# zju3dv/OnePose_Plus_Plus

Hardware: AMD Instinct MI355X
Metric: query images/sec (2D-3D match fwd) at 512x512 img x 5k pts (higher is better)
Workload: dtype f32 (operands as exact bf16 triples, f32 accumulate)

## Files before the change

### onepose_plus_plus_amd/build.py

```python
import hashlib
import os
import subprocess
import sys
from concurrent.futures import ThreadPoolExecutor

HERE = os.path.dirname(os.path.abspath(__file__))
CSRC = os.path.join(HERE, "csrc")
OBJ = os.path.join(HERE, "csrc", "_build")
LIB = os.path.join(HERE, "libopp_hip.so")
SOURCES = ["gemm_mfma.hip", "gemm_ss.hip", "enc_chain.hip", "enc_layer64.hip", "stem_direct.hip", "attention.hip", "full_attention.hip", "backbone.hip", "kpt.hip",
           "coarse_match.hip", "fine.hip", "pnp.hip", "pnp_batch.hip", "pnp_lo.hip", "pnp_lo_batch.hip", "pose_metrics.hip", "ingest.hip", "track.hip", "profile.hip", "bn_train.hip", "bankbuild.hip", "loss.hip", "linear_bwd.hip",
           "linattn_train.hip", "conv_bwd.hip", "train_misc.hip", "conv_tail.hip", "version.hip", "api.hip"]
HEADERS = ["opp_common.h", "opp_internal.h", "enc_frag.h", "pnp_math.h", "pnp_sample.h", "pnp_body.h", "pnp_batch.h", "pnp_lo_body.h", "pnp_lo_batch.h", os.path.join("..", "..", "include", "opp_hip.h")]
FLAGS = ["--offload-arch=gfx950", "-O3", "-std=c++17", "-fPIC", "-Wall", "-Wno-unused-function"]
SOURCE_FLAGS = {"conv_bwd.hip": ["-fno-slp-vectorize"], "gemm_mfma.hip": ["-fno-slp-vectorize"], "full_attention.hip": ["-fno-slp-vectorize"]}


def _hipcc():
    for cand in (os.environ.get("HIPCC"), "/opt/rocm/bin/hipcc", "hipcc"):
        if cand and (os.path.isabs(cand) and os.path.exists(cand) or not os.path.isabs(cand)):
            return cand
    return "hipcc"


def _max_jobs():
    if os.environ.get("MAX_JOBS", "").isdigit() and int(os.environ["MAX_JOBS"]) > 0:
        return int(os.environ["MAX_JOBS"])
    return len(os.sched_getaffinity(0)) if hasattr(os, "sched_getaffinity") else (os.cpu_count() or 4)


def source_hash():
    h = hashlib.sha256()
    for rel in sorted(SOURCES + HEADERS):
        path = os.path.join(CSRC, rel)
        if not os.path.exists(path):
            return None
        h.update(os.path.basename(rel).encode() + b"\0")
        with open(path, "rb") as f:
            h.update(f.read())
        h.update(b"\0")
    return h.hexdigest()


def _stale(target, deps):
    if not os.path.exists(target):
        return True
# ... 70 lines not shown
```

### onepose_plus_plus_amd/csrc/api.hip

```cpp
#include <math.h>
#include <stdarg.h>

#include <string>
#include <vector>

#include "../../include/opp_hip.h"
#include "opp_internal.h"

static thread_local char g_err[512] = "";
void opp_set_error(const char* fmt, ...) {
  va_list ap;
  va_start(ap, fmt);
  vsnprintf(g_err, sizeof(g_err), fmt, ap);
  va_end(ap);
}
extern "C" const char* opp_last_error(void) { return g_err; }
extern "C" int opp_version(void) { return 1; }

namespace {

inline int pad32(int c) { return (c + 31) / 32 * 32; }

inline int gemm_prec(const opp_config& cfg) {
  return cfg.gemm_precision == 3 ? OPP_PREC_BF16X3 : cfg.gemm_precision ? OPP_PREC_FP16X2 : OPP_PREC_FP32;
// ... 588 lines not shown
  }
};
bool conv_splits_by_shape(const ConvDesc& d, size_t pixels, int prec) {
  return prec == OPP_PREC_BF16X3 && opp_conv_splitk_by_shape((long long)pixels, d.cout_pad(), d.k_len());
}

inline bool asp_env_on() {
  const char* e = getenv("OPP_ASP");
  return e && e[0] == '1';
}
thread_local bool t_asp_on = false;
struct AspScope {
  bool prev;
  AspScope() : prev(t_asp_on) { t_asp_on = asp_env_on(); }
  explicit AspScope(bool on) : prev(t_asp_on) { t_asp_on = on; }
  ~AspScope() { t_asp_on = prev; }
};
bool conv_takes_split(const ConvDesc& d, int prec) {
  return t_asp_on && prec == OPP_PREC_BF16X3 && opp_conv_tail_grp(d.cin, d.ks) == 0 && !(t_conv_tail && d.w_tail != nullptr);
}
inline size_t split_row_bytes(int c_pad) { return (size_t)c_pad * 6; }

inline int conv_out(int in, int ks, int stride, int pad = -1) { return (in + 2 * (pad < 0 ? ks / 2 : pad) - ks) / stride + 1; }

struct ConvOpts {
  int tile_cfg = -1;
  int Bn = 1;
  bool raw = false;
  int pad = -1;
  int splitk_force = -1;
  const void* x3 = nullptr;
  void* y3 = nullptr;
};

int run_conv(const float* x, int Hin, int Win, const ConvDesc& d, int stride, const float* res, int res_mode, int act,
             float* y, hipStream_t s, int h2, const ConvOpts& o = ConvOpts()) {
  OppGemm g;
  const bool raw = o.raw;
  const bool a_split = o.x3 != nullptr && !raw && conv_takes_split(d, h2);
  OPP_CHECK_ARG(a_split || x != nullptr, "conv: no fp32 input for a convolution that cannot take the pre-split one");
  OPP_CHECK_ARG(o.y3 == nullptr || h2 == OPP_PREC_BF16X3, "conv: pre-split output is a bf16x3 feature");
  static const bool splitk_on = !(getenv("OPP_CONV_SPLITK") && getenv("OPP_CONV_SPLITK")[0] == '0');
  g.splitk_ws = splitk_on ? t_splitk_ws : nullptr;
  g.splitk_ws_floats = g.splitk_ws ? t_splitk_ws_floats : 0;
  g.splitk_force = o.splitk_force;
  g.nonfinite = t_status_flag;
  g.tile_policy = t_tile_policy;
  g.conv = 1;
  g.prec = h2;
  const float* h2s = raw ? d.h2s_train : d.h2s;
  g.h2_inv = (h2 == OPP_PREC_FP16X2 && h2s) ? h2s + 1 : nullptr;
  g.A0 = a_split ? static_cast<const float*>(o.x3) : x;
  g.a_split = a_split ? 1 : 0;
  g.C3 = o.y3;
  g.ld3 = (int)split_row_bytes(d.cout_pad());
  g.Bn = o.Bn;
  g.Hin = Hin;
  g.Win = Win;
  g.Cin = d.cin_pad();
  g.ksize = d.ks;
  g.stride = stride;
  g.pad = o.pad < 0 ? d.ks / 2 : o.pad;
  g.Hout = conv_out(Hin, d.ks, stride, g.pad);
  g.Wout = conv_out(Win, d.ks, stride, g.pad);
  g.W = raw ? d.w_train : d.w;
  g.K = d.k_len();
  g.tail_grp = opp_conv_tail_grp(d.cin, d.ks);
  g.ldw = (int)split_floats((size_t)g.K, h2);
  g.M = o.Bn * g.Hout * g.Wout;
  g.N = d.cout_pad();
  g.C = y;
  g.ldc = d.cout_pad();
  g.n_store = d.cout_pad();
  g.n_real = d.cout;
  g.bias = raw ? nullptr : d.bias;
  g.res_mode = res_mode;
  g.R = res;
  g.ldr = d.cout_pad();
  if (res_mode == OPP_RES_BILINEAR2X) {
    g.Hr = g.Hout / 2;
    g.Wr = g.Wout / 2;
    g.res_sy = g.Hout > 1 ? (float)(g.Hr - 1) / (float)(g.Hout - 1) : 0.f;
    g.res_sx = g.Wout > 1 ? (float)(g.Wr - 1) / (float)(g.Wout - 1) : 0.f;
  }
  g.act = act;
  g.alg_flops = 2.0 * (double)g.M * (double)d.cout * (double)(d.ks * d.ks * d.cin);
  const float* wt = raw ? d.w_tail_train : d.w_tail;
  if (t_conv_tail && h2 == OPP_PREC_BF16X3 && wt != nullptr && o.tile_cfg < 0) {
    OppGemm body = g;
    body.N = d.body_cols();
    body.n_store = d.body_cols();
    body.alg_flops = 2.0 * (double)g.M * (double)d.body_cols() * (double)(d.ks * d.ks * d.cin);
    OPP_TRY(opp_gemm_launch_cfg(body, o.tile_cfg, s));
    return opp_conv_tail(g, wt, d.body_cols(), d.tail_cols(), s);
  }
  return opp_gemm_launch_cfg(g, o.tile_cfg, s);
}

struct BlockTwins {
  const void* x3 = nullptr;
  void *tmp3 = nullptr, *y3 = nullptr;
};

int run_block(const float* x, int Hin, int Win, const BlockDesc& b, int stride, float* tmp, float* ds, float* y,
              hipStream_t s, int h2, const BlockTwins& tw = BlockTwins()) {
  const int Ho = Hin / stride, Wo = Win / stride;
  const bool t_split = tw.tmp3 != nullptr && conv_takes_split(b.conv2, h2);
  OPP_TRY(run_conv(x, Hin, Win, b.conv1, stride, nullptr, OPP_RES_NONE, OPP_ACT_RELU, t_split ? nullptr : tmp, s, h2,
                   {.x3 = tw.x3, .y3 = t_split ? tw.tmp3 : nullptr}));
  const float* shortcut = x;
  if (b.has_down) {
    OPP_TRY(run_conv(x, Hin, Win, b.down, stride, nullptr, OPP_RES_NONE, OPP_ACT_NONE, ds, s, h2, {.x3 = tw.x3}));
    shortcut = ds;
  }
  OPP_CHECK_ARG(shortcut != nullptr, "block: the shortcut needs the fp32 input map");
  return run_conv(t_split ? nullptr : tmp, Ho, Wo, b.conv2, 1, shortcut, OPP_RES_DIRECT, OPP_ACT_RELU, y, s, h2,
                  {.x3 = t_split ? tw.tmp3 : nullptr, .y3 = tw.y3});
}

struct BackboneBufs {
  float *col, *x0, *t1, *x1a, *x1, *t2, *ds2, *x2a, *x2, *t3, *ds3, *x3a, *x3, *l2, *u2, *x2o, *l1, *u1;
  float *sk1 = nullptr, *sk2 = nullptr;
  void *x0s = nullptr, *t1s = nullptr, *x1as = nullptr, *x1s = nullptr, *x2s = nullptr, *t3s = nullptr, *x3as = nullptr, *x3s = nullptr, *l2s = nullptr,
       *u2s = nullptr;
};

size_t plan_backbone(const opp_ctx* c, int B, int H, int W, bool infer, Arena& a, BackboneBufs& b) {
  const size_t p2 = (size_t)B * (H / 2) * (W / 2), p4 = (size_t)B * (H / 4) * (W / 4), p8 = (size_t)B * (H / 8) * (W / 8);
// ... 1683 lines not shown
```

### onepose_plus_plus_amd/csrc/gemm_mfma.hip

```cpp
#include <stdlib.h>

#include <mutex>
#include <type_traits>

#include <vector>

#include "opp_internal.h"

typedef float f32x16 __attribute__((ext_vector_type(16)));
typedef _Float16 f16x8 __attribute__((ext_vector_type(8)));
typedef __bf16 bf16x8 __attribute__((ext_vector_type(8)));
typedef __bf16 bf16x2 __attribute__((ext_vector_type(2)));
typedef float f32x2 __attribute__((ext_vector_type(2)));

namespace {

constexpr int lds_stride(int prec) { return prec == OPP_PREC_BF16X3 ? 52 : 36; }

__device__ __forceinline__ void opp_split4_b3(const float4 v, uint2& hi, uint2& mid, uint2& lo) {
  auto lvl = [](float a, float b, float& ra, float& rb) -> unsigned {
    const f32x2 t = {a, b};
    const unsigned p = __builtin_bit_cast(unsigned, __builtin_convertvector(t, bf16x2));
    ra = a - __uint_as_float(p << 16);
    rb = b - __uint_as_float(p & 0xffff0000u);
    return p;
  };
  float r0, r1, r2, r3, s0, s1, s2, s3, u0, u1, u2, u3;
  const unsigned h01 = lvl(v.x, v.y, r0, r1), h23 = lvl(v.z, v.w, r2, r3);
  const unsigned m01 = lvl(r0, r1, s0, s1), m23 = lvl(r2, r3, s2, s3);
  const unsigned l01 = lvl(s0, s1, u0, u1), l23 = lvl(s2, s3, u2, u3);
  hi = make_uint2(h01, h23);
  mid = make_uint2(m01, m23);
  lo = make_uint2(l01, l23);
}
__device__ __forceinline__ void opp_store_split4(void* base, size_t row_bytes_off, int col, const float4 v) {
  uint2 hi, mid, lo;
  opp_split4_b3(v, hi, mid, lo);
  char* p = static_cast<char*>(base) + row_bytes_off + (col >> 3) * 48 + (col & 7) * 2;
  *reinterpret_cast<uint2*>(p) = hi;
  *reinterpret_cast<uint2*>(p + 16) = mid;
  *reinterpret_cast<uint2*>(p + 32) = lo;
}

template <int BM, int BN, int WAVES_M, int WAVES_N, bool CONV, int ABL, int DEPTH, int PREC, bool ASP, bool KFOLD = false>
__device__ __forceinline__ void opp_gemm_body(const OppGemm& g) {
  constexpr bool H2 = PREC == OPP_PREC_FP16X2;
  constexpr bool H3 = PREC == OPP_PREC_BF16X3;
  constexpr int kLdsStride = lds_stride(PREC);
  constexpr int NT = WAVES_M * WAVES_N * 64;
  constexpr int TM = BM / WAVES_M / 32;
  constexpr int NT32 = BN / 32;
  constexpr int TN = (NT32 + WAVES_N - 1) / WAVES_N;
  constexpr bool kRagged = (NT32 % WAVES_N) != 0;
  static_assert(!ASP || (CONV && PREC == OPP_PREC_BF16X3 && (ABL == 0 || ABL >= 200)), "pre-split activations: bf16x3 convolutions only");
  constexpr int kAblMask = ABL >= 200 ? ABL - 200 : 0;
  constexpr bool kNoGload = ABL == 91 || (kAblMask & 1), kNoLdsSt = ABL == 92 || (kAblMask & 2), kNoBar = ABL == 93 || (kAblMask & 4),
                 kNoFrag = ABL == 94 || (kAblMask & 8);
  constexpr int A_LD = ASP ? (BM * 12 + NT - 1) / NT : BM * 8 / NT;
  constexpr bool kAFrac = ASP && (BM * 12) % NT != 0;
  constexpr int kBRowsLoad = (H3 && BN == 224) ? 208 : BN;
  constexpr int B_LD = H3 ? (kBRowsLoad * 12 + NT - 1) / NT : BN * 8 / NT;
  constexpr bool kBFrac = H3 && (kBRowsLoad * 12) % NT != 0;
  constexpr bool kRing = H3 && kRagged && !CONV;
  constexpr bool kM16 = H3 && CONV;
  constexpr int NB16 = kM16 ? kBRowsLoad / 16 : 1;
  constexpr int NBW = kM16 ? (NB16 + WAVES_N - 1) / WAVES_N : 1;
  constexpr bool kRoles = kM16 && BM == 128 && BN == 224 && WAVES_M == 2 && WAVES_N == 4;
// ... 1076 lines not shown
      if constexpr (decltype(vec_c)::value) return *reinterpret_cast<const vf4*>(p);
      return vf4{p[0], nval > 1 ? p[1] : 0.f, nval > 2 ? p[2] : 0.f, nval > 3 ? p[3] : 0.f};
    };
    auto epi_col = [&](int lc, int& col) __attribute__((always_inline)) -> bool {
      const int wn2 = lc / (JP * 32);
      const int j = ps * JP + (lc - wn2 * JP * 32) / 32;
      col = kM16 ? n0 + lc : n0 + wn2 * TN * 32 + j * 32 + (lc & 31);
      return !((!kM16 && (j >= TN || (kRagged && wn2 * TN + j >= NT32))) || col >= g.n_store);
    };
    vf4 bias_t = vf4{0.f, 0.f, 0.f, 0.f};
    if constexpr (kColFixed) {
      int col;
      if (g.bias && epi_col((tid % kRowQ) * 4, col)) bias_t = vec_ok ? ld4(std::true_type{}, g.bias + col, 4) : ld4(std::false_type{}, g.bias + col, g.n_store - col);
    }
    const bool row_masked = g.act == OPP_ACT_QKV && g.row_mask != nullptr;
    auto epi_load = [&](auto vec_c, auto m_c, int u, EpiItem& it) __attribute__((always_inline)) {
      constexpr int M = decltype(m_c)::value;
      constexpr bool direct = M == kRDirect, bilinear = CONV && M == kRBil;
      it.ok = false;
      if (u >= kUnits) return;
      const int lr = u / kRowQ;
      const int lc = (u - lr * kRowQ) * 4;
      it.row = m0 + lr;
      if (!epi_col(lc, it.col) || it.row >= g.M) return;
      it.ok = true;
      const int nval = g.n_store - it.col < 4 ? g.n_store - it.col : 4;
      it.cv = *reinterpret_cast<const vf4*>(Cs + lr * CS + lc);
      if constexpr (!kColFixed) {
        if (g.bias) it.bv = ld4(vec_c, g.bias + it.col, nval);
      }
      if (row_masked && it.row < g.row_mask_rows) it.rm = g.row_mask[it.row];
      if (direct) it.rd = ld4(vec_c, g.R + (size_t)it.row * g.ldr + it.col, nval);
      if (bilinear) {
#pragma clang fp contract(off)
        const int ox = it.row % g.Wout;
        const int t = it.row / g.Wout;
        const int oy = t % g.Hout;
        const int b = t / g.Hout;
        const float sy = g.res_sy * (float)oy;
        const float sx = g.res_sx * (float)ox;
        int y0 = (int)sy;
        if (y0 > g.Hr - 1) y0 = g.Hr - 1;
        int x0 = (int)sx;
        if (x0 > g.Wr - 1) x0 = g.Wr - 1;
        const int y1 = y0 + (y0 < g.Hr - 1 ? 1 : 0);
        const int x1 = x0 + (x0 < g.Wr - 1 ? 1 : 0);
        it.wy1 = fminf(fmaxf(sy - (float)y0, 0.f), 1.f);
        it.wx1 = fminf(fmaxf(sx - (float)x0, 0.f), 1.f);
        it.wy0 = 1.f - it.wy1;
        it.wx0 = 1.f - it.wx1;
        const int pb = b * g.Hr * g.Wr;
        it.r[0] = ld4(vec_c, g.R + (size_t)(pb + y0 * g.Wr + x0) * g.ldr + it.col, nval);
        it.r[1] = ld4(vec_c, g.R + (size_t)(pb + y0 * g.Wr + x1) * g.ldr + it.col, nval);
        it.r[2] = ld4(vec_c, g.R + (size_t)(pb + y1 * g.Wr + x0) * g.ldr + it.col, nval);
        it.r[3] = ld4(vec_c, g.R + (size_t)(pb + y1 * g.Wr + x1) * g.ldr + it.col, nval);
      }
    };
    auto epi_finish = [&](auto vec_c, auto m_c, auto w_c, const EpiItem& it) __attribute__((always_inline)) {
      constexpr int M = decltype(m_c)::value;
      constexpr bool direct = M == kRDirect, bilinear = CONV && M == kRBil;
      if (!it.ok) return;
      const int row = it.row, col = it.col;
      const int nval = g.n_store - col < 4 ? g.n_store - col : 4;
      float v[4] = {it.cv.x, it.cv.y, it.cv.z, it.cv.w};
      if (g.bias) {
        const vf4 bv = kColFixed ? bias_t : it.bv;
        v[0] += bv.x; v[1] += bv.y; v[2] += bv.z; v[3] += bv.w;
      }
      if (direct) {
        const vf4 rv = it.rd;
        v[0] += rv.x; v[1] += rv.y; v[2] += rv.z; v[3] += rv.w;
      } else if (bilinear) {
#pragma clang fp contract(off)
        const float a00[4] = {it.r[0].x, it.r[0].y, it.r[0].z, it.r[0].w}, a01[4] = {it.r[1].x, it.r[1].y, it.r[1].z, it.r[1].w};
        const float a10[4] = {it.r[2].x, it.r[2].y, it.r[2].z, it.r[2].w}, a11[4] = {it.r[3].x, it.r[3].y, it.r[3].z, it.r[3].w};
#pragma unroll
        for (int e = 0; e < 4; ++e) {
          const float top = it.wx0 * a00[e] + it.wx1 * a01[e];
          const float bot = it.wx0 * a10[e] + it.wx1 * a11[e];
          v[e] += it.wy0 * top + it.wy1 * bot;
        }
      }
      if (g.act == OPP_ACT_RELU) {
#pragma unroll
        for (int e = 0; e < 4; ++e) v[e] = v[e] < 0.f ? 0.f : v[e];
      } else if (g.act == OPP_ACT_LEAKY) {
#pragma unroll
        for (int e = 0; e < 4; ++e) v[e] = v[e] > 0.f ? v[e] : 0.01f * v[e];
      } else if (g.act == OPP_ACT_QKV) {
        if (col < g.qk_cols) {
#pragma unroll
          for (int e = 0; e < 4; ++e) v[e] = v[e] > 0.f ? v[e] + 1.f : __expf(v[e]);
        } else {
          const float vdiv = row < g.split_row ? g.s0 : g.s1;
#pragma unroll
          for (int e = 0; e < 4; ++e) v[e] = v[e] / vdiv;
        }
        if constexpr (decltype(w_c)::value) {
          if (row_masked && row < g.row_mask_rows) {
#pragma unroll
            for (int e = 0; e < 4; ++e) v[e] *= it.rm;
          }
        }
      }
      if constexpr (H3) {
        if (g.C3 != nullptr) opp_store_split4(g.C3, (size_t)row * g.ld3, col, make_float4(v[0], v[1], v[2], v[3]));
      }
      if (g.C == nullptr) return;
      float* cp = g.C + (size_t)row * g.ldc + col + (g.k_splits > 1 ? (size_t)blockIdx.y * g.split_stride : 0);
      if constexpr (decltype(vec_c)::value) {
        *reinterpret_cast<float4*>(cp) = make_float4(v[0], v[1], v[2], v[3]);
      } else {
        for (int e = 0; e < nval; ++e) cp[e] = v[e];
      }
    };
    constexpr int kWaitVm0 = 0x0F70;
    auto epi_batches = [&](auto vec_c, auto eb_c, auto m_c, auto w_c) __attribute__((always_inline)) {
      constexpr int EB = decltype(eb_c)::value;
      constexpr bool W = decltype(w_c)::value;
      if constexpr (!W) __builtin_amdgcn_s_waitcnt(kWaitVm0);
      for (int ub = tid; ub < kUnits; ub += NT * EB) {
        EpiItem it[EB];
// ... 490 lines not shown
```

### onepose_plus_plus_amd/csrc/opp_internal.h

```cpp
#pragma once
#include "opp_common.h"

enum {
  OPP_PROF_FIRST_NON_GEMM = 1000,
  OPP_PROF_LINATTN_KV = 1000,
  OPP_PROF_LINATTN_APPLY = 1001,
  OPP_PROF_CONF = 1002,
  OPP_PROF_FINE = 1003,
  OPP_PROF_LINATTN_SMALL = 1004,
  OPP_PROF_FINE_GATHER = 1005,
  OPP_PROF_FINE_HEAD = 1006,
  OPP_PROF_FOCAL_FWD = 1007,
  OPP_PROF_FOCAL_BWD = 1008,
  OPP_PROF_ENC_CHAIN = 1009,
  OPP_PROF_SCORE_SWEEP1 = 1010,
  OPP_PROF_SCORE_SWEEP2 = 1011,
  OPP_PROF_CONV_WGRAD = 1013,
  OPP_PROF_CONV_SPLITK = 1014,
  OPP_PROF_CONV_TAIL = 1017,
  OPP_PROF_LINATTN_REDUCE = 1016,
  OPP_PROF_SPLITK_EPILOGUE = 1015,
  OPP_PROF_SCORE_SS = 1012,
};
inline int opp_prof_gemm_symbol(int tile_cfg, int kind) { return kind * 256 + tile_cfg; }
struct OppProfScope {
  OppProfScope(int symbol, hipStream_t stream, double work);
  ~OppProfScope();
  OppProfScope(const OppProfScope&) = delete;
  OppProfScope& operator=(const OppProfScope&) = delete;

 private:
  hipStream_t stream_;
  long long slot_ = -1;
};

int opp_layernorm(const float* x, int ldx, const float* gamma, const float* beta, const float* res, int ldres,
                  float* out, int ldo, int rows, int C, float eps, hipStream_t stream);
int opp_linattn_chunks(int seg_len);
int opp_linattn_kv(const float* k, const float* v, int ld, int n_seg, int seg_len, int C, int D, float* kv_out,
                   float* ks_out, float* scratch, hipStream_t stream);
int opp_linattn_apply(const float* q, int ldq, const float* kv, const float* ks, float* out, int ldo, int n_seg,
                      int seg_len, int src_len, int C, int D, float eps, hipStream_t stream);
size_t opp_linattn_pair_scratch_floats(int len0, int len1);
int opp_linattn_kv_pair(const float* qkv, int ld, int len0, int len1, float* kv, float* ks, float* scratch,
                        hipStream_t stream);
void opp_linattn_chunk_parts(float* scratch, int len0, int len1, float** kv_part, float** ks_part);
int opp_linattn_reduce_chunks(int len0, int len1, float* kv, float* ks, float* scratch, hipStream_t stream);
size_t opp_focal_loss_ws_bytes(size_t n);
int opp_focal_loss_fwd(const float* conf, const short* gt, const float* weight, size_t n, float alpha, float gamma, double* sums,
                       void* ws, size_t ws_bytes, hipStream_t stream);
int opp_focal_loss_bwd(const float* conf, const short* gt, const float* weight, size_t n, float alpha, float gamma,
                       const float* scales, float* grad, hipStream_t stream);
int opp_focal_loss_fwd_ex(const float* conf, const void* gt, int gt_kind, const float* weight, const float* mask0, const float* mask1, int N, int L,
                          size_t n, float alpha, float gamma, double* sums, void* ws, size_t ws_bytes, hipStream_t stream);
// ... 61 lines not shown
  const float* rstat_max = nullptr;
  const float* rstat_sum = nullptr;
  const float* cstat_max = nullptr;
  const float* cstat_sum = nullptr;
  float* C = nullptr;
  int ldc = 0;
  float* part_best = nullptr;
  int* part_arg = nullptr;
  int* part_ties = nullptr;
  float* part_rowmax = nullptr;
  int a_bytes = 0, b_bytes = 0, vec_store = 0;
  int delay = 0;
  unsigned long long* dbg_ts = nullptr;
};
void opp_gemm_ss_debug_timestamps(void* buf, int mode);
int opp_gemm_ss_tile_rows();
int opp_gemm_ss_tile_cols();
int opp_gemm_ss(const OppGemmSS& g, hipStream_t stream);
size_t opp_linear_bwd_ws_bytes(int M, int N, int K, int prec);
int opp_linear_bwd(const float* dY, const float* X, const float* W, int M, int N, int K, float* dX, float* dW, int accumulate_dw, int prec,
                   void* ws, size_t ws_bytes, hipStream_t stream);
size_t opp_linattn_train_ws_bytes(int B, int L, int S, int H, int D);
int opp_linattn_train_fwd(const float* q, const float* k, const float* v, const float* q_mask, const float* kv_mask, int B, int L, int S, int H, int D,
                          float eps, float* out, float* kv, float* ks, void* ws, size_t ws_bytes, hipStream_t stream);
int opp_linattn_train_bwd(const float* q, const float* k, const float* v, const float* q_mask, const float* kv_mask, const float* kv, const float* ks,
                          const float* grad_out, int B, int L, int S, int H, int D, float eps, float* gq, float* gk, float* gv, void* ws,
                          size_t ws_bytes, hipStream_t stream);
bool opp_stem_direct_ok(int cout, int prec);
int opp_stem_direct(const float* img, int H, int W, const float* wsplit, const float* bias, float* out, int ldc, hipStream_t stream, void* out3 = nullptr,
                    int ld3 = 0);
size_t opp_conv_tail_weight_floats(int cin_pad, int ks);
int opp_pack_conv_tail(const float* w, const float* scale, int cout, int cin, int ks, int n0, int cin_pad, float* wt, hipStream_t stream);
int opp_conv_tail(const OppGemm& g, const float* wt, int n0, int ncols, hipStream_t stream);
int opp_fold_bn(const float* gamma, const float* beta, const float* mean, const float* var, float eps, int c,
                int c_pad, float* scale, float* shift, hipStream_t stream);
int opp_pack_conv(const float* w, const float* scale, int cout, int cin, int ks, int cout_pad, int cin_pad,
                  float* out, hipStream_t stream);
int opp_pack_stem(const float* w, const float* scale, int cout, float* out, hipStream_t stream);
int opp_stem_im2col(const float* img, int B, int H, int W, float* col, hipStream_t stream);
int opp_h2_split(const float* in, float* out, size_t n, float* scale2, hipStream_t stream);
int opp_b3_split(const float* in, float* out, size_t n, hipStream_t stream);
int opp_add(const float* a, const float* b, float* out, size_t n, hipStream_t stream);
int opp_pack_affine(const float* src, float fill, const float* scale1, float* out, int n, hipStream_t stream);
int opp_add_cat(const float* a, const float* b, size_t na, const float* c, size_t nc, float* out, hipStream_t stream);
int opp_transpose(const float* in, float* out, int batch, int R, int Cc, hipStream_t stream);
size_t opp_bn_train_scratch_bytes(int rows, int ld);
int opp_bn_train(const float* y, int rows, int ld, int C, const float* gamma, const float* beta, float eps, const float* res,
                 int act, float* out, float* stat_out, void* scratch, hipStream_t stream, float* save_mean = nullptr, float* save_invstd = nullptr);
size_t opp_conv_geo_entries(int P);
int opp_conv_geo(int B, int Ho, int Wo, int Hin, int Win, int ks, int stride, int pad, void* geo, hipStream_t stream);
size_t opp_conv_wgrad_ws_bytes(int P, int cout_pad, int cin_pad, int ks);
int opp_conv_wgrad(const float* dY, int ldy, const float* X, int ldx, size_t x_pixels, const void* geo, int P, int Win, int ks, int cout, int cin,
                   float* dW, int accumulate, void* ws, size_t ws_bytes, hipStream_t stream);
int opp_conv_flip_transpose(const float* w, int cout, int cin, int ks, float* out, hipStream_t stream);
int opp_conv_dilate2(const float* dy, int B, int Ho, int Wo, int ld, float* z, hipStream_t stream);
size_t opp_bn_bwd_scratch_bytes(int rows, int ld);
int opp_bn_backward(const float* dy, const float* y, const float* raw, int rows, int ld, int C, int act, const float* gamma, const float* mean,
                    const float* invstd, float* draw, float* dres, float* dgamma, float* dbeta, int accumulate, void* scratch, hipStream_t stream);
int opp_upsample2x_backward(const float* g, int B, int Hr, int Wr, int ld, float* dr, int accumulate, hipStream_t stream);
int opp_ln_forward(const float* x, const float* gamma, const float* beta, const float* res, int rows, int C, float eps, float* y, float* mean,
                   float* rstd, hipStream_t stream);
size_t opp_ln_backward_ws_bytes(int rows, int C);
int opp_ln_backward(const float* g, const float* x, const float* gamma, const float* mean, const float* rstd, int rows, int C, float* dx,
                    float* dgamma, float* dbeta, void* ws, size_t ws_bytes, hipStream_t stream);
size_t opp_lse_ws_bytes(int B, int N, int L);
int opp_dual_softmax_lse(const float* S, int B, int N, int L, float* lse_row, float* lse_col, float* conf, void* ws, size_t ws_bytes,
// ... 38 lines not shown
```

Measured before the change: 597.0.

## Add dedicated short-K 1x1 convolution MFMA kernel for bf16x3 convs

Result: no change. 596.5 (-0.1%).

```diff
diff --git a/onepose_plus_plus_amd/build.py b/onepose_plus_plus_amd/build.py
--- a/onepose_plus_plus_amd/build.py
+++ b/onepose_plus_plus_amd/build.py
@@ -10,8 +10,8 @@
 LIB = os.path.join(HERE, "libopp_hip.so")
 SOURCES = ["gemm_mfma.hip", "gemm_ss.hip", "enc_chain.hip", "enc_layer64.hip", "stem_direct.hip", "attention.hip", "full_attention.hip", "backbone.hip", "kpt.hip",
            "coarse_match.hip", "fine.hip", "pnp.hip", "pnp_batch.hip", "pnp_lo.hip", "pnp_lo_batch.hip", "pose_metrics.hip", "ingest.hip", "track.hip", "profile.hip", "bn_train.hip", "bankbuild.hip", "loss.hip", "linear_bwd.hip",
-           "linattn_train.hip", "conv_bwd.hip", "train_misc.hip", "conv_tail.hip", "version.hip", "api.hip"]
-HEADERS = ["opp_common.h", "opp_internal.h", "enc_frag.h", "pnp_math.h", "pnp_sample.h", "pnp_body.h", "pnp_batch.h", "pnp_lo_body.h", "pnp_lo_batch.h", os.path.join("..", "..", "include", "opp_hip.h")]
+           "linattn_train.hip", "conv_bwd.hip", "train_misc.hip", "conv_tail.hip", "conv1x1.hip", "version.hip", "api.hip"]
+HEADERS = ["opp_common.h", "opp_internal.h", "conv_epilogue.h", "split_b3.h", "enc_frag.h", "pnp_math.h", "pnp_sample.h", "pnp_body.h", "pnp_batch.h", "pnp_lo_body.h", "pnp_lo_batch.h", os.path.join("..", "..", "include", "opp_hip.h")]
 FLAGS = ["--offload-arch=gfx950", "-O3", "-std=c++17", "-fPIC", "-Wall", "-Wno-unused-function"]
 SOURCE_FLAGS = {"conv_bwd.hip": ["-fno-slp-vectorize"], "gemm_mfma.hip": ["-fno-slp-vectorize"], "full_attention.hip": ["-fno-slp-vectorize"]}
 
diff --git a/onepose_plus_plus_amd/csrc/api.hip b/onepose_plus_plus_amd/csrc/api.hip
--- a/onepose_plus_plus_amd/csrc/api.hip
+++ b/onepose_plus_plus_amd/csrc/api.hip
@@ -644,6 +644,11 @@
   const void* x3 = nullptr;
   void* y3 = nullptr;
 };
+
+inline int conv1x1_mode() {
+  const char* v = getenv("OPP_CONV1X1");
+  return v && (v[0] == '0' || v[0] == '1') ? v[0] - '0' : -1;
+}
 
 int run_conv(const float* x, int Hin, int Win, const ConvDesc& d, int stride, const float* res, int res_mode, int act,
              float* y, hipStream_t s, int h2, const ConvOpts& o = ConvOpts()) {
@@ -706,6 +711,10 @@
     OPP_TRY(opp_gemm_launch_cfg(body, o.tile_cfg, s));
     return opp_conv_tail(g, wt, d.body_cols(), d.tail_cols(), s);
   }
+  const int c1_mode = conv1x1_mode();
+  if (o.tile_cfg < 0 && !raw && o.x3 == nullptr && o.y3 == nullptr && h2 == OPP_PREC_BF16X3 && c1_mode != 0 &&
+      (c1_mode == 1 || g.M < opp_conv1x1_max_pixels()) && opp_conv1x1_takes(g))
+    return opp_conv1x1_launch(g, s);
   return opp_gemm_launch_cfg(g, o.tile_cfg, s);
 }
 
diff --git a/onepose_plus_plus_amd/csrc/conv1x1.hip b/onepose_plus_plus_amd/csrc/conv1x1.hip
--- /dev/null
+++ b/onepose_plus_plus_amd/csrc/conv1x1.hip
@@ -0,0 +1,276 @@
+#include <stdlib.h>
+
+#include <type_traits>
+
+#include "conv_epilogue.h"
+#include "opp_internal.h"
+#include "split_b3.h"
+
+namespace {
+
+typedef __bf16 bf16x8 __attribute__((ext_vector_type(8)));
+typedef float f32x4 __attribute__((ext_vector_type(4)));
+typedef unsigned int u32x4 __attribute__((ext_vector_type(4)));
+
+constexpr int kTileM = 64;
+constexpr int kNT = 256;
+constexpr int kRowF = 52;
+constexpr int kFill = 4;
+constexpr int kChunkF = kTileM * kRowF;
+constexpr unsigned kOob = 0x80000000u;
+
+__device__ __forceinline__ int c1_kswz(int r) { return ((r >> 2) ^ (r >> 3)) & 1; }
+__device__ __forceinline__ float4 c1_bload(const __amdgpu_buffer_rsrc_t r, unsigned voff, unsigned soff) {
+  const u32x4 v = __builtin_amdgcn_raw_buffer_load_b128(r, (int)voff, (int)soff, 0);
+  return make_float4(__uint_as_float(v.x), __uint_as_float(v.y), __uint_as_float(v.z), __uint_as_float(v.w));
+}
+__device__ __forceinline__ bf16x8 c1_b8(const float4& v) { return *reinterpret_cast<const bf16x8*>(&v); }
+
+__global__ __launch_bounds__(kNT, 3) void conv1x1_kernel(const OppGemm g, const int nb_comp) {
+  __shared__ __attribute__((aligned(16))) float As[kFill * kChunkF];
+
+  const int tid = threadIdx.x;
+  const int lane = tid & 63;
+  const int wave = __builtin_amdgcn_readfirstlane(tid >> 6);
+  int tile = blockIdx.x;
+  {
+    const int nb = gridDim.x, q = nb >> 3, r = nb & 7;
+    const int xcd = blockIdx.x & 7, idx = blockIdx.x >> 3;
+    tile = (xcd < r ? xcd * (q + 1) : r * (q + 1) + (xcd - r) * q) + idx;
+  }
+  const int m0 = tile * kTileM;
+  const int nk = g.K >> 5;
+
+  const int role = (wave + tile) & 3;
+  const int wg_base = nb_comp / (int)gridDim.y, wg_rem = nb_comp % (int)gridDim.y;
+  const int wg_nb = wg_base + ((int)blockIdx.y < wg_rem ? 1 : 0);
+  const int wg_cb0 = (int)blockIdx.y * wg_base + ((int)blockIdx.y < wg_rem ? (int)blockIdx.y : wg_rem);
+  const int nb_base = wg_nb >> 2, nb_rem = wg_nb & 3;
+  const int nbw = nb_base + (role < nb_rem ? 1 : 0);
+  const int cb0 = wg_cb0 + role * nb_base + (role < nb_rem ? role : nb_rem);
+
+  const int kq = tid & 7, lrow = tid >> 3;
+  unsigned a_base[2];
+  int a_lds[2];
+#pragma unroll
+  for (int h = 0; h < 2; ++h) {
+    const int lr = lrow + 32 * h;
+    const int r = m0 + lr;
+    const int ox = r % g.Wout;
+    const int t = r / g.Wout;
+    const int oy = t % g.Hout;
+    const int b = t / g.Hout;
+    a_base[h] = r < g.M ? (unsigned)(((b * g.Hin + oy * g.stride) * g.Win + ox * g.stride) * g.Cin + kq * 4) * 4u : kOob;
+    a_lds[h] = lr * kRowF + ((kq >> 1) ^ c1_kswz(lr)) * 12 + (kq & 1) * 2;
+  }
+  const __amdgpu_buffer_rsrc_t ra = __builtin_amdgcn_make_buffer_rsrc(const_cast<float*>(g.A0), 0, g.a0_bytes, 0x00020000);
+  const __amdgpu_buffer_rsrc_t rw = __builtin_amdgcn_make_buffer_rsrc(const_cast<float*>(g.W), 0, g.w_bytes, 0x00020000);
+  auto stage = [&](int c0, auto grp_c) __attribute__((always_inline)) {
+    constexpr int G = decltype(grp_c)::value;
+#pragma unroll
+    for (int c1 = 0; c1 < kFill; c1 += G) {
+      float4 v[G][2];
+#pragma unroll
+      for (int ci = 0; ci < G; ++ci)
+#pragma unroll
+        for (int h = 0; h < 2; ++h) v[ci][h] = c1_bload(ra, (c0 + c1 + ci < nk ? a_base[h] : kOob) + (unsigned)(c0 + c1 + ci) * 128u, 0);
+#pragma unroll
+      for (int ci = 0; ci < G; ++ci)
+#pragma unroll
+        for (int h = 0; h < 2; ++h) {
+          uint2 hi, mid, lo;
+          opp_split4_b3(v[ci][h], hi, mid, lo);
+          float* dst = As + (c1 + ci) * kChunkF + a_lds[h];
+          *reinterpret_cast<uint2*>(dst) = hi;
+          *reinterpret_cast<uint2*>(dst + 4) = mid;
+          *reinterpret_cast<uint2*>(dst + 8) = lo;
+        }
+    }
+  };
+
+  const int l15 = lane & 15, kg = lane >> 4;
+  const int f16off = l15 * kRowF + ((kg ^ c1_kswz(l15)) * 3) * 4;
+  const unsigned w_voff = (unsigned)((cb0 * 16 + l15) * g.ldw) * 4u + (unsigned)kg * 48u;
+  const unsigned w_blk = (unsigned)(16 * g.ldw) * 4u;
+
+  auto body = [&](auto nbw_c) __attribute__((always_inline)) {
+    constexpr int NBW = decltype(nbw_c)::value;
+    constexpr int NBA = NBW > 0 ? NBW : 1;
+    constexpr int WD = NBW <= 1 ? 8 : NBW == 2 ? 3 : NBW == 3 ? 2 : 1;
+    f32x4 acc[4][NBA];
+    float4 wf[WD][NBA][3];
+    float4 af[2][3];
+#pragma unroll
+    for (int i = 0; i < 4; ++i)
+#pragma unroll
+      for (int j = 0; j < NBA; ++j) acc[i][j] = f32x4{0.f, 0.f, 0.f, 0.f};
+    auto load_w = [&](int slot, int j, int c) {
+      const int cc = c < nk ? c : nk - 1;
+#pragma unroll
+      for (int p = 0; p < 3; ++p) wf[slot][j][p] = c1_bload(rw, w_voff, (unsigned)j * w_blk + (unsigned)cc * 192u + (unsigned)p * 16u);
+    };
+    auto read_a = [&](int slot, const float* img, int i) {
+#pragma unroll
+      for (int p = 0; p < 3; ++p) af[slot][p] = *reinterpret_cast<const float4*>(img + i * 16 * kRowF + p * 4);
+    };
+    auto chunk = [&](auto c_c) __attribute__((always_inline)) {
+      constexpr int CC = decltype(c_c)::value, SLOT = CC % WD;
+      constexpr int PA[6] = {2, 0, 1, 1, 0, 0};
+      constexpr int PB[6] = {0, 2, 1, 0, 1, 0};
+      const float* img = As + (CC & (kFill - 1)) * kChunkF + f16off;
+      if (NBW > 0) read_a(0, img, 0);
+#pragma unroll
+      for (int j = 0; j < NBW; ++j) {
+#pragma unroll
+        for (int i = 0; i < 4; ++i) {
+          if (i < 3 || j + 1 < NBW) read_a((i + 1) & 1, img, (i + 1) & 3);
+#pragma unroll
+          for (int pr = 0; pr < 6; ++pr)
+            acc[i][j] = __builtin_amdgcn_mfma_f32_16x16x32_bf16(c1_b8(wf[SLOT][j][PB[pr]]), c1_b8(af[i & 1][PA[pr]]), acc[i][j], 0, 0, 0);
+        }
+        if constexpr (CC + WD < 8) load_w(SLOT, j, CC + WD);
+        __builtin_amdgcn_sched_barrier(0);
+      }
+    };
+
+#pragma unroll
+    for (int sl = 0; sl < WD; ++sl)
+#pragma unroll
+      for (int j = 0; j < NBW; ++j) load_w(sl, j, sl);
+    stage(0, std::integral_constant<int, 4>{});
+    __syncthreads();
+    chunk(std::integral_constant<int, 0>{});
+    chunk(std::integral_constant<int, 1>{});
+    chunk(std::integral_constant<int, 2>{});
+    chunk(std::integral_constant<int, 3>{});
+    if (nk > kFill) {
+      __syncthreads();
+      stage(kFill, std::integral_constant<int, 2>{});
+      __syncthreads();
+      chunk(std::integral_constant<int, 4>{});
+      if (nk > 5) chunk(std::integral_constant<int, 5>{});
+      if (nk > 6) chunk(std::integral_constant<int, 6>{});
+      if (nk > 7) chunk(std::integral_constant<int, 7>{});
+    }
+
+    const opp_vf4 zero4 = opp_vf4{0.f, 0.f, 0.f, 0.f};
+    const opp_vf4 none4[4] = {zero4, zero4, zero4, zero4};
+#pragma unroll
+    for (int j = 0; j < NBW; ++j) {
+      const opp_vf4 bv = g.bias ? *reinterpret_cast<const opp_vf4*>(g.bias + (cb0 + j) * 16 + kg * 4) : zero4;
+#pragma unroll
+      for (int i = 0; i < 4; ++i) {
+        float v[4] = {acc[i][j][0], acc[i][j][1], acc[i][j][2], acc[i][j][3]};
+        opp_epi_bias_res4<false, false>(v, g.bias != nullptr, bv, zero4, none4, 0.f, 0.f, 0.f, 0.f);
+        acc[i][j] = f32x4{v[0], v[1], v[2], v[3]};
+      }
+    }
+    auto finish = [&](auto bil_c) __attribute__((always_inline)) {
+      constexpr bool BIL = decltype(bil_c)::value;
+      auto item = [&](const f32x4 a, const opp_vf4 (&r)[4], const OppBil2x& t, int row, int col) {
+        float v[4] = {a[0], a[1], a[2], a[3]};
+        opp_epi_bias_res4<false, BIL>(v, false, zero4, zero4, r, t.wx0, t.wx1, t.wy0, t.wy1);
+        opp_epi_act4(v, g.act);
+        if (row < g.M) *reinterpret_cast<float4*>(g.C + (size_t)row * g.ldc + col) = make_float4(v[0], v[1], v[2], v[3]);
+      };
+      auto taps = [&](opp_vf4 (&r)[4], const OppBil2x& t, int col) {
+        if constexpr (BIL) {
+          r[0] = *reinterpret_cast<const opp_vf4*>(g.R + (size_t)t.p00 * g.ldr + col);
+          r[1] = *reinterpret_cast<const opp_vf4*>(g.R + (size_t)t.p01 * g.ldr + col);
+          r[2] = *reinterpret_cast<const opp_vf4*>(g.R + (size_t)t.p10 * g.ldr + col);
+          r[3] = *reinterpret_cast<const opp_vf4*>(g.R + (size_t)t.p11 * g.ldr + col);
+        }
+      };
+      auto geo = [&](int i, OppBil2x& t) {
+        const int row = m0 + i * 16 + l15;
+        if constexpr (BIL) opp_epi_bil2x(g, row < g.M ? row : g.M - 1, t);
+      };
+      constexpr int JP = NBW > 0 ? (NBW + 1) / 2 : 1, NBATCH = NBW > 0 ? 4 * JP : 0;
+      OppBil2x t[2] = {};
+      opp_vf4 r[2][2][4];
+      auto request = [&](int b) {
+        const int i = b / JP, j0 = (b % JP) * 2;
+        if (b % JP == 0) geo(i, t[i & 1]);
+#pragma unroll
+        for (int jj = 0; jj < 2; ++jj)
+          if (j0 + jj < NBW) taps(r[b & 1][jj], t[i & 1], (cb0 + j0 + jj) * 16 + kg * 4);
+      };
+      if (NBATCH > 0) request(0);
+#pragma unroll
+      for (int b = 0; b < NBATCH; ++b) {
+        if (b + 1 < NBATCH) request(b + 1);
+        const int i = b / JP, j0 = (b % JP) * 2;
+#pragma unroll
+        for (int jj = 0; jj < 2; ++jj)
+          if (j0 + jj < NBW) item(acc[i][j0 + jj], r[b & 1][jj], t[i & 1], m0 + i * 16 + l15, (cb0 + j0 + jj) * 16 + kg * 4);
+      }
+      if (blockIdx.y == 0) {
+        const int nb_store = g.n_store >> 4;
+        for (int e = nb_comp + wave; e < nb_store; e += 4) {
+          const int col = e * 16 + kg * 4;
+          const opp_vf4 bz = g.bias ? *reinterpret_cast<const opp_vf4*>(g.bias + col) : zero4;
+          for (int i = 0; i < 4; ++i) {
+            OppBil2x tz = {};
+            geo(i, tz);
+            opp_vf4 rz[4];
+            taps(rz, tz, col);
+            float v[4] = {0.f, 0.f, 0.f, 0.f};
+            opp_epi_bias_res4<false, false>(v, g.bias != nullptr, bz, zero4, none4, 0.f, 0.f, 0.f, 0.f);
+            item(f32x4{v[0], v[1], v[2], v[3]}, rz, tz, m0 + i * 16 + l15, col);
+          }
+        }
+      }
+    };
+    if (g.res_mode == OPP_RES_BILINEAR2X) finish(std::true_type{});
+    else finish(std::false_type{});
+  };
+
+  if (nbw == 4) body(std::integral_constant<int, 4>{});
+  else if (nbw == 3) body(std::integral_constant<int, 3>{});
+  else if (nbw == 2) body(std::integral_constant<int, 2>{});
+  else if (nbw == 1) body(std::integral_constant<int, 1>{});
+  else body(std::integral_constant<int, 0>{});
+}
+
+bool al16(const void* p) { return (reinterpret_cast<uintptr_t>(p) & 15) == 0; }
+
+}
+
+int opp_conv1x1_max_pixels() { return 4096; }
+
+bool opp_conv1x1_takes(const OppGemm& g) {
+  if (!g.conv || g.ksize != 1 || g.pad != 0 || (g.stride != 1 && g.stride != 2) || g.prec != OPP_PREC_BF16X3) return false;
+  if (g.a_split || g.C3 != nullptr || g.C == nullptr || g.Bn != 1 || g.k_splits > 1 || g.splitk_force > 0 || g.tail_grp != 0) return false;
+  if (g.K != g.Cin || g.K % 32 != 0 || g.K < 4 * 32 || g.K > 8 * 32) return false;
+  if (g.N <= 0 || g.N % 16 != 0 || g.N > g.n_store || g.n_store > 256 || g.n_store % 16 != 0 || g.ldc < g.n_store || g.ldc % 4 != 0) return false;
+  if (g.res_mode != OPP_RES_NONE && g.res_mode != OPP_RES_BILINEAR2X) return false;
+  if (g.act != OPP_ACT_NONE && g.act != OPP_ACT_RELU && g.act != OPP_ACT_LEAKY) return false;
+  if (g.out_mul != 1.f || g.out_div != 1.f || g.ln_gamma || g.stat_rowmax || g.col_mask || g.row_mask) return false;
+  if (g.M <= 0 || g.M != g.Hout * g.Wout || (size_t)g.M * (size_t)g.ldc >= (1ull << 31)) return false;
+  if ((size_t)g.Hin * g.Win * g.Cin * 4 >= (1ull << 31) || (size_t)g.N * g.ldw * 4 >= (1ull << 31) || g.ldw * 2 < g.K * 3 || g.ldw % 4 != 0) return false;
+  if ((g.Hout - 1) * g.stride >= g.Hin || (g.Wout - 1) * g.stride >= g.Win) return false;
+  if (!al16(g.A0) || !al16(g.W) || !al16(g.C) || !al16(g.bias)) return false;
+  if (g.res_mode == OPP_RES_BILINEAR2X) {
+    if (g.R == nullptr || !al16(g.R) || g.ldr % 4 != 0 || g.ldr < g.n_store || g.Hr <= 0 || g.Wr <= 0) return false;
+    const uintptr_t r0 = reinterpret_cast<uintptr_t>(g.R), r1 = r0 + ((size_t)(g.Hr * g.Wr - 1) * g.ldr + g.n_store) * 4;
+    const uintptr_t c0 = reinterpret_cast<uintptr_t>(g.C), c1 = c0 + ((size_t)(g.M - 1) * g.ldc + g.n_store) * 4;
+    if (!(r1 <= c0 || c1 <= r0)) return false;
+  }
+  return true;
+}
+
+int opp_conv1x1_launch(const OppGemm& g_in, hipStream_t stream) {
+  OPP_CHECK_ARG(opp_conv1x1_takes(g_in), "conv1x1: not a convolution of the short-K kernel");
+  OppGemm g = g_in;
+  g.a0_bytes = (unsigned)((size_t)g.Hin * g.Win * g.Cin * 4);
+  g.w_bytes = (unsigned)((size_t)g.N * g.ldw * 4);
+  const int n_real = g.n_real > 0 && g.n_real < g.N ? g.n_real : g.N;
+  const int nb_comp = (n_real + 15) / 16;
+  OppProfScope prof(OPP_PROF_CONV1X1, stream, g.alg_flops > 0.0 ? g.alg_flops : 2.0 * (double)g.M * (double)g.N * (double)g.K);
+  const int tiles_m = opp_cdiv(g.M, kTileM);
+  int col_split = 1;
+  while (col_split < 4 && tiles_m * col_split < 512 && nb_comp >= 8 * col_split) col_split *= 2;
+  hipLaunchKernelGGL(conv1x1_kernel, dim3(tiles_m, col_split), dim3(kNT), 0, stream, g, nb_comp);
+  OPP_CHECK_LAUNCH("conv1x1_kernel");
+  return OPP_OK;
+}
diff --git a/onepose_plus_plus_amd/csrc/conv_epilogue.h b/onepose_plus_plus_amd/csrc/conv_epilogue.h
--- /dev/null
+++ b/onepose_plus_plus_amd/csrc/conv_epilogue.h
@@ -0,0 +1,66 @@
+#pragma once
+#include "opp_common.h"
+
+#ifdef __HIPCC__
+typedef float opp_vf4 __attribute__((ext_vector_type(4)));
+
+struct OppBil2x {
+  int p00, p01, p10, p11;
+  float wx0, wx1, wy0, wy1;
+};
+__device__ __forceinline__ void opp_epi_bil2x(const OppGemm& g, int row, OppBil2x& t) {
+#pragma clang fp contract(off)
+  const int ox = row % g.Wout;
+  const int q = row / g.Wout;
+  const int oy = q % g.Hout;
+  const int b = q / g.Hout;
+  const float sy = g.res_sy * (float)oy;
+  const float sx = g.res_sx * (float)ox;
+  int y0 = (int)sy;
+  if (y0 > g.Hr - 1) y0 = g.Hr - 1;
+  int x0 = (int)sx;
+  if (x0 > g.Wr - 1) x0 = g.Wr - 1;
+  const int y1 = y0 + (y0 < g.Hr - 1 ? 1 : 0);
+  const int x1 = x0 + (x0 < g.Wr - 1 ? 1 : 0);
+  t.wy1 = fminf(fmaxf(sy - (float)y0, 0.f), 1.f);
+  t.wx1 = fminf(fmaxf(sx - (float)x0, 0.f), 1.f);
+  t.wy0 = 1.f - t.wy1;
+  t.wx0 = 1.f - t.wx1;
+  const int pb = b * g.Hr * g.Wr;
+  t.p00 = pb + y0 * g.Wr + x0;
+  t.p01 = pb + y0 * g.Wr + x1;
+  t.p10 = pb + y1 * g.Wr + x0;
+  t.p11 = pb + y1 * g.Wr + x1;
+}
+
+template <bool DIRECT, bool BILINEAR>
+__device__ __forceinline__ void opp_epi_bias_res4(float (&v)[4], bool has_bias, const opp_vf4 bv, const opp_vf4 rd, const opp_vf4 (&r)[4], float wx0,
+                                                  float wx1, float wy0, float wy1) {
+  if (has_bias) {
+    v[0] += bv.x; v[1] += bv.y; v[2] += bv.z; v[3] += bv.w;
+  }
+  if (DIRECT) {
+    v[0] += rd.x; v[1] += rd.y; v[2] += rd.z; v[3] += rd.w;
+  } else if (BILINEAR) {
+#pragma clang fp contract(off)
+    const float a00[4] = {r[0].x, r[0].y, r[0].z, r[0].w}, a01[4] = {r[1].x, r[1].y, r[1].z, r[1].w};
+    const float a10[4] = {r[2].x, r[2].y, r[2].z, r[2].w}, a11[4] = {r[3].x, r[3].y, r[3].z, r[3].w};
+#pragma unroll
+    for (int e = 0; e < 4; ++e) {
+      const float top = wx0 * a00[e] + wx1 * a01[e];
+      const float bot = wx0 * a10[e] + wx1 * a11[e];
+      v[e] += wy0 * top + wy1 * bot;
+    }
+  }
+}
+
+__device__ __forceinline__ void opp_epi_act4(float (&v)[4], int act) {
+  if (act == OPP_ACT_RELU) {
+#pragma unroll
+    for (int e = 0; e < 4; ++e) v[e] = v[e] < 0.f ? 0.f : v[e];
+  } else if (act == OPP_ACT_LEAKY) {
+#pragma unroll
+    for (int e = 0; e < 4; ++e) v[e] = v[e] > 0.f ? v[e] : 0.01f * v[e];
+  }
+}
+#endif
diff --git a/onepose_plus_plus_amd/csrc/gemm_mfma.hip b/onepose_plus_plus_amd/csrc/gemm_mfma.hip
--- a/onepose_plus_plus_amd/csrc/gemm_mfma.hip
+++ b/onepose_plus_plus_amd/csrc/gemm_mfma.hip
@@ -5,7 +5,9 @@
 
 #include <vector>
 
+#include "conv_epilogue.h"
 #include "opp_internal.h"
+#include "split_b3.h"
 
 typedef float f32x16 __attribute__((ext_vector_type(16)));
 typedef _Float16 f16x8 __attribute__((ext_vector_type(8)));
@@ -17,22 +19,6 @@
 
 constexpr int lds_stride(int prec) { return prec == OPP_PREC_BF16X3 ? 52 : 36; }
 
-__device__ __forceinline__ void opp_split4_b3(const float4 v, uint2& hi, uint2& mid, uint2& lo) {
-  auto lvl = [](float a, float b, float& ra, float& rb) -> unsigned {
-    const f32x2 t = {a, b};
-    const unsigned p = __builtin_bit_cast(unsigned, __builtin_convertvector(t, bf16x2));
-    ra = a - __uint_as_float(p << 16);
-    rb = b - __uint_as_float(p & 0xffff0000u);
-    return p;
-  };
-  float r0, r1, r2, r3, s0, s1, s2, s3, u0, u1, u2, u3;
-  const unsigned h01 = lvl(v.x, v.y, r0, r1), h23 = lvl(v.z, v.w, r2, r3);
-  const unsigned m01 = lvl(r0, r1, s0, s1), m23 = lvl(r2, r3, s2, s3);
-  const unsigned l01 = lvl(s0, s1, u0, u1), l23 = lvl(s2, s3, u2, u3);
-  hi = make_uint2(h01, h23);
-  mid = make_uint2(m01, m23);
-  lo = make_uint2(l01, l23);
-}
 __device__ __forceinline__ void opp_store_split4(void* base, size_t row_bytes_off, int col, const float4 v) {
   uint2 hi, mid, lo;
   opp_split4_b3(v, hi, mid, lo);
@@ -1175,28 +1161,16 @@
       if (row_masked && it.row < g.row_mask_rows) it.rm = g.row_mask[it.row];
       if (direct) it.rd = ld4(vec_c, g.R + (size_t)it.row * g.ldr + it.col, nval);
       if (bilinear) {
-#pragma clang fp contract(off)
-        const int ox = it.row % g.Wout;
-        const int t = it.row / g.Wout;
-        const int oy = t % g.Hout;
-        const int b = t / g.Hout;
-        const float sy = g.res_sy * (float)oy;
-        const float sx = g.res_sx * (float)ox;
-        int y0 = (int)sy;
-        if (y0 > g.Hr - 1) y0 = g.Hr - 1;
-        int x0 = (int)sx;
-        if (x0 > g.Wr - 1) x0 = g.Wr - 1;
-        const int y1 = y0 + (y0 < g.Hr - 1 ? 1 : 0);
-        const int x1 = x0 + (x0 < g.Wr - 1 ? 1 : 0);
-        it.wy1 = fminf(fmaxf(sy - (float)y0, 0.f), 1.f);
-        it.wx1 = fminf(fmaxf(sx - (float)x0, 0.f), 1.f);
-        it.wy0 = 1.f - it.wy1;
-        it.wx0 = 1.f - it.wx1;
-        const int pb = b * g.Hr * g.Wr;
-        it.r[0] = ld4(vec_c, g.R + (size_t)(pb + y0 * g.Wr + x0) * g.ldr + it.col, nval);
-        it.r[1] = ld4(vec_c, g.R + (size_t)(pb + y0 * g.Wr + x1) * g.ldr + it.col, nval);
-        it.r[2] = ld4(vec_c, g.R + (size_t)(pb + y1 * g.Wr + x0) * g.ldr + it.col, nval);
-        it.r[3] = ld4(vec_c, g.R + (size_t)(pb + y1 * g.Wr + x1) * g.ldr + it.col, nval);
+        OppBil2x t;
+        opp_epi_bil2x(g, it.row, t);
+        it.wy1 = t.wy1;
+        it.wx1 = t.wx1;
+        it.wy0 = t.wy0;
+        it.wx0 = t.wx0;
+        it.r[0] = ld4(vec_c, g.R + (size_t)t.p00 * g.ldr + it.col, nval);
+        it.r[1] = ld4(vec_c, g.R + (size_t)t.p01 * g.ldr + it.col, nval);
+        it.r[2] = ld4(vec_c, g.R + (size_t)t.p10 * g.ldr + it.col, nval);
+        it.r[3] = ld4(vec_c, g.R + (size_t)t.p11 * g.ldr + it.col, nval);
       }
     };
     auto epi_finish = [&](auto vec_c, auto m_c, auto w_c, const EpiItem& it) __attribute__((always_inline)) {
@@ -1206,31 +1180,9 @@
       const int row = it.row, col = it.col;
       const int nval = g.n_store - col < 4 ? g.n_store - col : 4;
       float v[4] = {it.cv.x, it.cv.y, it.cv.z, it.cv.w};
-      if (g.bias) {
-        const vf4 bv = kColFixed ? bias_t : it.bv;
-        v[0] += bv.x; v[1] += bv.y; v[2] += bv.z; v[3] += bv.w;
-      }
-      if (direct) {
-        const vf4 rv = it.rd;
-        v[0] += rv.x; v[1] += rv.y; v[2] += rv.z; v[3] += rv.w;
-      } else if (bilinear) {
-#pragma clang fp contract(off)
-        const float a00[4] = {it.r[0].x, it.r[0].y, it.r[0].z, it.r[0].w}, a01[4] = {it.r[1].x, it.r[1].y, it.r[1].z, it.r[1].w};
-        const float a10[4] = {it.r[2].x, it.r[2].y, it.r[2].z, it.r[2].w}, a11[4] = {it.r[3].x, it.r[3].y, it.r[3].z, it.r[3].w};
-#pragma unroll
-        for (int e = 0; e < 4; ++e) {
-          const float top = it.wx0 * a00[e] + it.wx1 * a01[e];
-          const float bot = it.wx0 * a10[e] + it.wx1 * a11[e];
-          v[e] += it.wy0 * top + it.wy1 * bot;
-        }
-      }
-      if (g.act == OPP_ACT_RELU) {
-#pragma unroll
-        for (int e = 0; e < 4; ++e) v[e] = v[e] < 0.f ? 0.f : v[e];
-      } else if (g.act == OPP_ACT_LEAKY) {
-#pragma unroll
-        for (int e = 0; e < 4; ++e) v[e] = v[e] > 0.f ? v[e] : 0.01f * v[e];
-      } else if (g.act == OPP_ACT_QKV) {
+      opp_epi_bias_res4<direct, bilinear>(v, g.bias != nullptr, kColFixed ? bias_t : it.bv, it.rd, it.r, it.wx0, it.wx1, it.wy0, it.wy1);
+      opp_epi_act4(v, g.act);
+      if (g.act == OPP_ACT_QKV) {
         if (col < g.qk_cols) {
 #pragma unroll
           for (int e = 0; e < 4; ++e) v[e] = v[e] > 0.f ? v[e] + 1.f : __expf(v[e]);
diff --git a/onepose_plus_plus_amd/csrc/opp_internal.h b/onepose_plus_plus_amd/csrc/opp_internal.h
--- a/onepose_plus_plus_amd/csrc/opp_internal.h
+++ b/onepose_plus_plus_amd/csrc/opp_internal.h
@@ -20,6 +20,7 @@
   OPP_PROF_CONV_TAIL = 1017,
   OPP_PROF_LINATTN_REDUCE = 1016,
   OPP_PROF_SPLITK_EPILOGUE = 1015,
+  OPP_PROF_CONV1X1 = 1018,
   OPP_PROF_SCORE_SS = 1012,
 };
 inline int opp_prof_gemm_symbol(int tile_cfg, int kind) { return kind * 256 + tile_cfg; }
@@ -147,6 +148,9 @@
 size_t opp_conv_tail_weight_floats(int cin_pad, int ks);
 int opp_pack_conv_tail(const float* w, const float* scale, int cout, int cin, int ks, int n0, int cin_pad, float* wt, hipStream_t stream);
 int opp_conv_tail(const OppGemm& g, const float* wt, int n0, int ncols, hipStream_t stream);
+bool opp_conv1x1_takes(const OppGemm& g);
+int opp_conv1x1_max_pixels();
+int opp_conv1x1_launch(const OppGemm& g, hipStream_t stream);
 int opp_fold_bn(const float* gamma, const float* beta, const float* mean, const float* var, float eps, int c,
                 int c_pad, float* scale, float* shift, hipStream_t stream);
 int opp_pack_conv(const float* w, const float* scale, int cout, int cin, int ks, int cout_pad, int cin_pad,
diff --git a/onepose_plus_plus_amd/csrc/split_b3.h b/onepose_plus_plus_amd/csrc/split_b3.h
--- /dev/null
+++ b/onepose_plus_plus_amd/csrc/split_b3.h
@@ -0,0 +1,23 @@
+#pragma once
+#include "opp_common.h"
+
+#ifdef __HIPCC__
+__device__ __forceinline__ void opp_split4_b3(const float4 v, uint2& hi, uint2& mid, uint2& lo) {
+  typedef __bf16 b2_t __attribute__((ext_vector_type(2)));
+  typedef float f2_t __attribute__((ext_vector_type(2)));
+  auto lvl = [](float a, float b, float& ra, float& rb) -> unsigned {
+    const f2_t t = {a, b};
+    const unsigned p = __builtin_bit_cast(unsigned, __builtin_convertvector(t, b2_t));
+    ra = a - __uint_as_float(p << 16);
+    rb = b - __uint_as_float(p & 0xffff0000u);
+    return p;
+  };
+  float r0, r1, r2, r3, s0, s1, s2, s3, u0, u1, u2, u3;
+  const unsigned h01 = lvl(v.x, v.y, r0, r1), h23 = lvl(v.z, v.w, r2, r3);
+  const unsigned m01 = lvl(r0, r1, s0, s1), m23 = lvl(r2, r3, s2, s3);
+  const unsigned l01 = lvl(s0, s1, u0, u1), l23 = lvl(s2, s3, u2, u3);
+  hi = make_uint2(h01, h23);
+  mid = make_uint2(m01, m23);
+  lo = make_uint2(l01, l23);
+}
+#endif
```
